# barronalex/Tacotron

Hardware: AMD Instinct MI355X
Metric: mel-frames/sec (train step, batch=32 r=2) (higher is better)
Workload: dtype f32

## Files before the change

### include/taco_hip.h

```cpp
#ifndef TACO_HIP_H
#define TACO_HIP_H

#include <stddef.h>
#include <stdint.h>

#ifdef __cplusplus
extern "C" {
#endif
#pragma GCC visibility push(default)

#define TACO_VERSION 120

#define TACO_OK 0
#define TACO_EINVAL (-1)
#define TACO_ELAUNCH (-2)
#define TACO_ENOTFOUND (-3)

#define TACO_ACT_NONE 0
#define TACO_ACT_RELU 1
#define TACO_ACT_SIGMOID 2
#define TACO_ACT_TANH 3

typedef struct TacoShape {
  int32_t B;
// ... 109 lines not shown
                  float* grads, void* workspace, void* stream);

int taco_infer(const TacoShape* shape, const float* params, const int32_t* text, const int32_t* text_length,
               const int32_t* speaker,
               float* seq2seq_output, float* output, float* alignments, void* workspace, void* stream);

typedef struct TacoStopRule {
  int32_t end_offset;
  int32_t hold;
  int32_t min_steps;
  int32_t reserved;
} TacoStopRule;

int taco_infer_stop(const TacoShape* shape, const float* params, const int32_t* text, const int32_t* text_length,
                    const int32_t* speaker, const TacoStopRule* rule, float* seq2seq_output, float* output, float* alignments,
                    int32_t* lengths, void* workspace, void* stream);

#define TACO_ALIGNMENT_MAX_TD 16384
#define TACO_ALIGNMENT_MAX_TT 16384
int taco_alignment_scores(const float* alignments, const int32_t* text_length, const int32_t* steps, int max_jump,
                          int32_t* counts, float* means, int B, int Td, int Tt, void* stream);

#define TACO_ALIGN_PATH_MAX_TD   16384
#define TACO_ALIGN_PATH_MAX_TT   4096
#define TACO_ALIGN_PATH_MAX_JUMP 15
int64_t taco_alignment_path_workspace_bytes(int B, int Td, int Tt);
int taco_alignment_path(const float* alignments, const int32_t* text_length, const int32_t* steps, int max_jump,
                        int32_t* path, int32_t* dur, int32_t* counts, float* mass, void* workspace,
                        int B, int Td, int Tt, void* stream);

int taco_frames_active(const float* x, float floor, int32_t* n, int B, int F, int C, void* stream);

#define TACO_DTW_MAX_FRAMES 1024
#define TACO_DTW_MAX_K 32
#define TACO_DTW_MAX_C 128
int64_t taco_frame_dtw_workspace_bytes(int B, int Fa, int Fb, int K);
int taco_frame_dtw(const float* a, const int32_t* na, const float* b, const int32_t* nb, const float* basis, float* cost,
                   int32_t* steps, void* workspace, int B, int Fa, int Fb, int C, int K, void* stream);

int64_t taco_frame_dtw_path_workspace_bytes(int B, int Fa, int Fb, int K);
int taco_frame_dtw_path(const float* a, const int32_t* na, const float* b, const int32_t* nb, const float* basis, float* cost,
                        int32_t* steps, int32_t* path_a, int32_t* path_b, void* workspace, int B, int Fa, int Fb, int C, int K,
                        void* stream);

int taco_clip_adam_step(float* params, const float* grads, float* m, float* v, int64_t n, float lr, float cap,
                        int64_t step, float* scratch, float* gnorm_out, void* stream);

int taco_clip_adam_step_guarded(float* params, const float* grads, float* m, float* v, int64_t n, float lr, float cap,
                                int64_t step, float* scratch, float* gnorm_out, const int32_t* err_words, void* stream);
int taco_clear_error(const TacoShape* shape, int train, void* workspace, void* stream);

int taco_decoder_mode(int mode);

int taco_grad_segments(const TacoShape* shape, int64_t* bounds);
int taco_wait_grad_segment(int seg, void* stream);
int taco_debug_spin(int blocks, int threads, int lds_bytes, int usec, void* stream);

int taco_debug_clock_probe(long long* out3, int iters, void* stream);

int taco_debug_fabric_probe(long long* out32, void* gran4k, const void* scratch, long long scratch_bytes, int iters, void* stream);

int taco_denorm_unframe(const float* output, const float* stft_mean, const float* stft_std, float* spec, float* mag_t,
                        int B, int Td, int r, int C, void* stream);

#define TACO_STRETCH_ONE        65536
#define TACO_STRETCH_MIN_STEP   16384
#define TACO_STRETCH_MAX_STEP   262144
#define TACO_STRETCH_MAX_FRAMES 8192
int taco_frames_stretch(const float* mag_t, const int32_t* frames, int frames_per_unit, const int32_t* step_q,
                        float* out, int32_t* frames_out, int B, int C, int F, int Fo, void* stream);

#define TACO_PITCH_ONE        65536
#define TACO_PITCH_MIN_STEP   32768
#define TACO_PITCH_MAX_STEP   131072
#define TACO_PITCH_MAX_LIFTER 64
#define TACO_PITCH_FLOOR      1e-8f
int taco_frames_pitch(const float* mag_t, const int32_t* frames, int frames_per_unit, const int32_t* step_q, int lifter,
                      float* out, int B, int C, int F, void* stream);

int taco_path_curve(const int32_t* path, const int32_t* values, int frames_per_step, int32_t fill, int32_t* curve, int B, int Td,
                    int Tt, void* stream);
int taco_frames_stretch_curve(const float* mag_t, const int32_t* frames, int frames_per_unit, const int32_t* dur_q, float* out,
                              int32_t* frames_out, int32_t* src, int B, int C, int F, int Fo, void* stream);
int taco_frames_pitch_curve(const float* mag_t, const int32_t* frames, int frames_per_unit, const int32_t* step_q, int lifter,
                            float* out, int B, int C, int F, void* stream);

#define TACO_SHARPEN_FIRST    2
#define TACO_SHARPEN_MIN_BETA -1.0f
#define TACO_SHARPEN_MAX_BETA 1.0f
int taco_frames_sharpen(const float* mag_t, const int32_t* frames, int frames_per_unit, float beta, int lifter, float* out, int B,
                        int C, int F, void* stream);
int64_t taco_frames_cepstats_workspace_bytes(int B, int C, int F, int lifter);
int taco_frames_cepstats(const float* mag_t, const int32_t* frames, int frames_per_unit, int lifter, double* sums, int32_t* count,
                         void* workspace, int B, int C, int F, void* stream);

#define TACO_F0_MAX_LAGS 512
int taco_frames_f0(const float* mag_t, const int32_t* frames, int frames_per_unit, const float* weight, const float* gain,
                   int lag_min, int lag_max, float ratio, float threshold, float* period, float* strength, float* acf,
                   int B, int C, int F, void* stream);

int taco_f0_stats(const float* period, const float* other, const int32_t* frames, int frames_per_unit, float* stats, int B, int F,
                  void* stream);

#define TACO_F0_MAX_CAND 15
int64_t taco_f0_viterbi_workspace_bytes(int B, int L, int F, int K);
int taco_f0_viterbi(const float* acf, const int32_t* frames, int frames_per_unit, const float* bias, const float* lg, int lag_min,
// ... 76 lines not shown
```

### tacotron_amd/csrc/gemm.hip

```cpp
#include <algorithm>

#include "bf16x3.h"
#include "common.h"
#include "kernels.h"

namespace {

constexpr int BK = 16;

__device__ __forceinline__ float4 sel4(bool ok, const float4 t) {
  return make_float4(ok ? t.x : 0.f, ok ? t.y : 0.f, ok ? t.z : 0.f, ok ? t.w : 0.f);
}

struct RowInfo {
  int m;
  int t;
  bool ok;
};

template <int WM, int WN, bool VA, bool VB>
__global__ __launch_bounds__(256) void conv_gemm_kernel(ConvGemmBatch batch) {
  constexpr int BM = 64 * WM, BN = 64 * WN;
  constexpr int LDS_A = BM + 4, LDS_B = BN + 4;
  constexpr int A_PER = BM / 64;
  constexpr int B_PER = BN / 64;
  const ConvGemmProblem& P = batch.p[blockIdx.z];
  const int m0 = blockIdx.x * BM, n0 = blockIdx.y * BN;
  if (m0 >= P.M || n0 >= P.N) return;

  __shared__ __attribute__((aligned(16))) float As[2][BK][LDS_A];
  __shared__ __attribute__((aligned(16))) float Bs[2][BK][LDS_B];

  const int tid = threadIdx.x, lane = tid & 63, wave = tid >> 6;
  const int wm = wave >> 1, wn = wave & 1;

  const int a_kq = tid & 3;
  const int a_row = tid >> 2;
  RowInfo ar[A_PER];
#pragma unroll
  for (int i = 0; i < A_PER; ++i) {
    int m = m0 + a_row + 64 * i;
    ar[i].m = m;
    ar[i].ok = m < P.M;
    ar[i].t = ar[i].ok ? (m % P.T) : 0;
  }
  constexpr int B_COLS4 = BN / 4;
  const int b_c4 = tid % B_COLS4;
  const int b_k = tid / B_COLS4;
  constexpr int B_KSTEP = 256 / B_COLS4;

  const int ktiles = (P.K + BK - 1) / BK;
  const int nit = P.taps * ktiles;

// ... 381 lines not shown
      if (kk + 2 < BK) {
#pragma unroll
        for (int i = 0; i < WM; ++i) a[nxt][i] = As[buf][kk + 2 + lk][wm * (32 * WM) + i * 32 + li];
#pragma unroll
        for (int j = 0; j < WN; ++j) b[nxt][j] = Bs[buf][kk + 2 + lk][wn * (32 * WN) + j * 32 + li];
      }
#pragma unroll
      for (int i = 0; i < WM; ++i)
#pragma unroll
        for (int j = 0; j < WN; ++j)
          acc[i][j] = __builtin_amdgcn_mfma_f32_32x32x2f32(a[cur][i], b[cur][j], acc[i][j], 0, 0, 0);
    }
    if (it + 1 < nit) store_tile(buf ^ 1);
    __syncthreads();
  }

  if constexpr (BX) {
#pragma unroll
    for (int i = 0; i < WM; ++i)
#pragma unroll
      for (int j = 0; j < WN; ++j) acc[i][j] += acc_lo[i][j];
  }
#pragma unroll
  for (int i = 0; i < WM; ++i) {
#pragma unroll
    for (int j = 0; j < WN; ++j) {
      const int n = n0 + wn * (32 * WN) + j * 32 + li;
      if (n >= P.N) continue;
#pragma unroll
      for (int e = 0; e < 16; ++e) {
        const int k = k0 + wm * (32 * WM) + i * 32 + (e & 3) + 8 * (e >> 2) + 4 * lk;
        if (k >= P.K) continue;
        atomicAdd(&W[(int64_t)k * P.ldw + n], acc[i][j][e]);
      }
    }
  }
  if (do_bias) {
    float* cs = &As[0][0][0];
    float4 t = make_float4(0.f, 0.f, 0.f, 0.f);
#pragma unroll
    for (int i = 0; i < B_PER; ++i) { t.x += bsum[i].x; t.y += bsum[i].y; t.z += bsum[i].z; t.w += bsum[i].w; }
    __syncthreads();
    *reinterpret_cast<float4*>(&cs[b_r * LDS_B + b_c4 * 4]) = t;
    __syncthreads();
    float* db = P.dbias + (int64_t)bz * P.N;
    for (int i = tid; i < BN; i += 256) {
      float c = 0.f;
      for (int r = 0; r < B_RSTEP; ++r) c += cs[r * LDS_B + i];
      if (n0 + i < P.N) atomicAdd(&db[n0 + i], c);
    }
  }
}

__device__ __forceinline__ void tn_xcd_order(int L, int per, int gz, bool on, int& t, int& z) {
  const int zfull = gz & ~7;
  if (on && L < per * zfull) {
    const int x = L & 7, s = L >> 3;
    const int g = s / per;
    z = x + 8 * g;
    t = s - g * per;
  } else {
    z = L / per;
    t = L - z * per;
  }
}

template <int WM, int WN, bool VA, bool VB, bool BX = false>
__global__ __launch_bounds__(256) void gemm_tn_kernel(GemmTnArgs P) {
  const int gx = gridDim.x, per = gx * gridDim.y;
  int t, z;
  tn_xcd_order(blockIdx.x + gx * (blockIdx.y + gridDim.y * blockIdx.z), per, gridDim.z, P.xcd != 0, t, z);
  const int by = t / gx;
  gemm_tn_body<WM, WN, VA, VB, BX>(P, t - by * gx, by, z);
}

template <bool BX>
__global__ __launch_bounds__(256) void gemm_tn_batch_kernel(GemmTnBatch B) {
  int pi = 0;
  for (int i = 1; i < B.n; ++i)
    if ((int)blockIdx.x >= B.first[i]) pi = i;
  const GemmTnArgs& P = B.p[pi];
  const int rel = blockIdx.x - B.first[pi];
  const int gx = B.gx[pi], per = gx * B.gy[pi], gz = P.batch * P.taps * P.splits;
  if (rel >= per * gz) return;
  int t, z;
  tn_xcd_order(rel, per, gz, P.xcd != 0, t, z);
  const int by = t / gx;
  gemm_tn_body<1, 1, true, true, BX>(P, t - by * gx, by, z);
}

__global__ void gemm_naive_kernel(ConvGemmProblem P) {
  const int64_t idx = (int64_t)blockIdx.x * blockDim.x + threadIdx.x;
  if (idx >= (int64_t)P.M * P.N) return;
  const int m = (int)(idx / P.N), n = (int)(idx % P.N);
  const int t = m % P.T;
  float acc = 0.f;
  for (int tap = 0; tap < P.taps; ++tap) {
    const int st = t + tap - P.pad_l;
    if (st < 0 || st >= P.T) continue;
    const float* a = P.A + (int64_t)(m + tap - P.pad_l) * P.lda;
    const float* w = P.W + (int64_t)tap * P.K * P.ldw + n;
    for (int k = 0; k < P.K; ++k) acc = fmaf(a[k], w[(int64_t)k * P.ldw], acc);
  }
  if (P.bias) acc += P.bias[n];
  P.C[(int64_t)m * P.ldc + n] = apply_act(acc, P.act);
}

inline bool aligned16(const void* p) { return (reinterpret_cast<uintptr_t>(p) & 15) == 0; }

}

void conv_gemm_set_flags(ConvGemmProblem& p) {
  p.flags = 0;
  if (p.Nld <= 0) p.Nld = (p.N % 4 == 0) ? p.N : 0;
  if (p.lda % 4 == 0 && aligned16(p.A) && p.K % 4 == 0) p.flags |= 1;
  if (p.ldw % 4 == 0 && aligned16(p.W) && ((int64_t)p.K * p.ldw) % 4 == 0 && p.Nld > 0 && p.Nld % 4 == 0 && p.Nld <= p.ldw)
    p.flags |= 2;
}

template <int WM, int WN>
static void dispatch_nn(int flags, dim3 grid, hipStream_t s, ConvGemmBatch& batch) {
  switch (flags & 3) {
    case 3: TACO_KLAUNCH((conv_gemm_kernel<WM, WN, true, true>), grid, dim3(256), 0, s, batch); break;
    case 1: TACO_KLAUNCH((conv_gemm_kernel<WM, WN, true, false>), grid, dim3(256), 0, s, batch); break;
    case 2: TACO_KLAUNCH((conv_gemm_kernel<WM, WN, false, true>), grid, dim3(256), 0, s, batch); break;
    default: TACO_KLAUNCH((conv_gemm_kernel<WM, WN, false, false>), grid, dim3(256), 0, s, batch); break;
  }
}

int launch_conv_gemm_batch(ConvGemmBatch& batch, hipStream_t stream) {
  TACO_REQUIRE(batch.n >= 1 && batch.n <= kMaxGemmBatch, "conv_gemm: batch size %d out of range", batch.n);
  int maxM = 0, maxN = 0, flags = 3;
  double work = 0;
  for (int i = 0; i < batch.n; ++i) {
    ConvGemmProblem& p = batch.p[i];
    TACO_REQUIRE(p.A && p.W && p.C, "conv_gemm: null operand");
    TACO_REQUIRE(p.M > 0 && p.N > 0 && p.K > 0 && p.taps > 0 && p.T > 0, "conv_gemm: bad dims M=%d N=%d K=%d taps=%d T=%d",
                 p.M, p.N, p.K, p.taps, p.T);
    TACO_REQUIRE(p.M % p.T == 0, "conv_gemm: M (%d) must be a multiple of T (%d)", p.M, p.T);
    conv_gemm_set_flags(p);
    flags &= p.flags;
// ... 75 lines not shown
          ConvGemmProblem& r = b.p[c];
          r = ConvGemmProblem();
          r.A = p.A; r.lda = p.lda; r.W = p.W; r.ldw = p.ldw; r.Nld = p.Nld; r.C = slabs + c * mn; r.ldc = p.N;
          r.M = p.M; r.N = p.N; r.K = p.K; r.taps = p.taps; r.T = p.T; r.pad_l = p.pad_l; r.act = TACO_ACT_NONE;
          r.it0 = c * per;
          r.it1 = std::min(nit, (c + 1) * per);
          conv_gemm_set_flags(r);
        }
        const int pslot = taco_prof_begin(2, stream);
        taco_prof_label(2, pslot, "nn-ksplit S=%d M=%d N=%d K=%d taps=%d", bestS, p.M, p.N, p.K, p.taps);
        const int rc = launch_conv_gemm2(b, stream, true);
        if (rc == TACO_OK) {
          const int64_t total4 = mn / 4;
          const int grid = (int)((total4 + 255) / 256 > 2048 ? 2048 : (total4 + 255) / 256);
          TACO_KLAUNCH(conv_gemm_tapsum_kernel, dim3(grid), dim3(256), 0, stream, p, slabs, bestS);
          taco_prof_end(2, pslot, stream, 2.0 * p.M * p.N * p.K * p.taps);
          TACO_LAUNCH_CHECK("conv_gemm2 k-split");
          return TACO_OK;
        }
        taco_prof_cancel(2, pslot, stream);
        if (rc != TACO_ENOTFOUND) return rc;
      }
    }
  }
  const double tiles64 = (double)cdiv(p.M, 64) * cdiv(p.N, 64);
  if (!slabs || p.taps < 2 || p.taps > kMaxGemmBatch || p.N % 4 != 0 || p.atomic_out || tiles64 > 320 || p.K < 512)
    return launch_conv_gemm(p, stream);
  ConvGemmBatch b;
  b.n = p.taps;
  const int64_t slab = (int64_t)p.M * p.N;
  for (int t = 0; t < p.taps; ++t) {
    ConvGemmProblem q;
    q.A = p.A; q.lda = p.lda; q.W = p.W + (int64_t)t * p.K * p.ldw; q.ldw = p.ldw; q.Nld = p.Nld;
    q.C = slabs + t * slab; q.ldc = p.N;
    q.M = p.M; q.N = p.N; q.K = p.K; q.taps = 1; q.T = p.T; q.pad_l = p.pad_l - t;
    q.act = TACO_ACT_NONE;
    b.p[t] = q;
  }
  TACO_TRY(launch_conv_gemm_batch(b, stream));
  const int64_t total4 = slab / 4;
  const int grid = (int)((total4 + 255) / 256 > 2048 ? 2048 : (total4 + 255) / 256);
  TACO_KLAUNCH(conv_gemm_tapsum_kernel, dim3(grid), dim3(256), 0, stream, p, slabs, p.taps);
  TACO_LAUNCH_CHECK("conv_gemm_tapsum");
  return TACO_OK;
}

int launch_conv_gemm(const ConvGemmProblem& p, hipStream_t stream) {
  ConvGemmBatch b;
  b.n = 1;
  b.p[0] = p;
  return launch_conv_gemm_batch(b, stream);
}

template <int WM, int WN>
static void dispatch_tn(int flags, dim3 grid, hipStream_t s, const GemmTnArgs& a) {
  switch (flags & 3) {
    case 3:
      if (env_bf16x() && a.chunk <= bf16x_max_chain()) TACO_KLAUNCH((gemm_tn_kernel<WM, WN, true, true, true>), grid, dim3(256), 0, s, a);
      else TACO_KLAUNCH((gemm_tn_kernel<WM, WN, true, true>), grid, dim3(256), 0, s, a);
      break;
    case 1: TACO_KLAUNCH((gemm_tn_kernel<WM, WN, true, false>), grid, dim3(256), 0, s, a); break;
    case 2: TACO_KLAUNCH((gemm_tn_kernel<WM, WN, false, true>), grid, dim3(256), 0, s, a); break;
    default: TACO_KLAUNCH((gemm_tn_kernel<WM, WN, false, false>), grid, dim3(256), 0, s, a); break;
  }
}

static int tn_block_target() {
  const int x = sw_int<SW_TN_BLOCKS>();
  return x > 0 ? x : 3072;
}

static int plan_gemm_tn(GemmTnArgs& a, bool force_small, dim3& grid, int64_t group_tiles = 0) {
  a.flags = 0;
  if (a.Nld <= 0) a.Nld = (a.N % 4 == 0) ? a.N : 0;
  const int64_t lim31 = (int64_t)1 << 31;
  if (a.lda % 4 == 0 && aligned16(a.A) && a.strideA % 4 == 0 && a.K % 4 == 0 && ((int64_t)a.M + a.taps + 48) * a.lda * 4 < lim31)
    a.flags |= 1;
  if (a.ldy % 4 == 0 && aligned16(a.Y) && a.strideY % 4 == 0 && a.Nld > 0 && a.Nld % 4 == 0 && a.Nld <= a.ldy &&
      ((int64_t)a.M + 16) * a.ldy * 4 < lim31)
    a.flags |= 2;
  const bool merge_taps = sw_on<SW_TN_MERGE_TAPS>();
  if (merge_taps && a.ktap == 0 && (a.flags & 1) && a.taps > 1 && a.taps <= 17 && a.K % 64 != 0 && a.pad_l <= 16 && a.taps - 1 - a.pad_l <= 16) {
    a.ktap = a.K;
    a.K *= a.taps;
    a.taps = 1;
  }
  const int force_bm = sw_int<SW_TN_BM>(), big_tiles = sw_int<SW_TN_BIG_TILES>();
  bool big = !force_small && (int64_t)cdiv(a.K, 128) * cdiv(a.N, 128) * a.taps * a.batch >= big_tiles && a.K >= 128 && a.N >= 128;
  if (!force_small && force_bm == 128 && a.K >= 128 && a.N >= 128) big = true;
  if (force_bm == 64) big = false;
  const int bm = big ? 128 : 64;
  const int64_t tiles = (int64_t)cdiv(a.K, bm) * cdiv(a.N, bm) * a.taps * a.batch;
  const int64_t fill = group_tiles > tiles ? group_tiles : tiles;
  int splits = taco_deterministic() ? 1 : (int)((tn_block_target() + fill - 1) / fill);
  const int max_splits = a.M >= 1280 ? cdiv(a.M, 320) : cdiv(a.M, 64);
  if (splits > max_splits) splits = max_splits;
  if (splits < 1) splits = 1;
  int chunk = cdiv(a.M, splits);
  chunk = cdiv(chunk, BK) * BK;
  splits = cdiv(a.M, chunk);
  a.splits = splits;
  a.chunk = chunk;
  grid = dim3(cdiv(a.K, bm), cdiv(a.N, bm), a.batch * a.taps * splits);
  a.xcd = sw_int<SW_TN_XCD>();
  return bm;
}

int launch_gemm_tn(GemmTnArgs a, bool zero_first, hipStream_t stream) {
  TACO_REQUIRE(a.A && a.Y && a.W, "gemm_tn: null operand");
  TACO_REQUIRE(a.M > 0 && a.N > 0 && a.K > 0 && a.taps > 0 && a.T > 0 && a.batch > 0, "gemm_tn: bad dims");
  TACO_REQUIRE(a.M % a.T == 0, "gemm_tn: M (%d) must be a multiple of T (%d)", a.M, a.T);
// ... 31 lines not shown
  TACO_REQUIRE(b.n >= 0 && b.n <= kMaxTnBatch, "gemm_tn_batch: %d problems out of range", b.n);
  GemmTnBatch grouped;
  int blocks = 0;
  GemmTnArgs big[kMaxTnBatch];
  int nbig = 0;
  double big_flops = 0;
  int64_t group_tiles = 0;
  for (int i = 0; i < b.n; ++i) {
    dim3 grid;
    GemmTnArgs probe = b.p[i];
    if (probe.A && probe.M > 0 && probe.N > 0 && probe.K > 0 && probe.taps > 0 && probe.batch > 0 && !gemm_tn2_eligible(probe) &&
        plan_gemm_tn(probe, false, grid) == 64 && probe.flags == 3)
      group_tiles += (int64_t)grid.x * grid.y * probe.taps * probe.batch;
  }
  for (int i = 0; i < b.n; ++i) {
    GemmTnArgs a = b.p[i];
    TACO_REQUIRE(a.A && a.Y && a.W, "gemm_tn_batch: null operand");
    TACO_REQUIRE(a.M > 0 && a.N > 0 && a.K > 0 && a.taps > 0 && a.T > 0 && a.batch > 0 && a.M % a.T == 0, "gemm_tn_batch: bad dims");
    if (gemm_tn2_eligible(a)) {
      big[nbig++] = a;
      big_flops += 2.0 * a.M * a.N * a.K * a.taps;
      continue;
    }
    dim3 grid;
    GemmTnArgs probe = a;
    const int bm = plan_gemm_tn(probe, false, grid, group_tiles);
    if (bm == 128 || probe.flags != 3) {
      TACO_TRY(launch_gemm_tn(a, false, stream));
      continue;
    }
    const int j = grouped.n++;
    grouped.p[j] = probe;
    grouped.first[j] = blocks;
    grouped.gx[j] = (int)grid.x;
    grouped.gy[j] = (int)grid.y;
    blocks += (int)(grid.x * grid.y * grid.z);
    blocks = (blocks + 7) & ~7;
  }
  if (nbig > 0) {
    const int pslot = taco_prof_begin(2, stream);
    TACO_TRY(launch_gemm_tn2(big, nbig, stream));
    taco_prof_end(2, pslot, stream, big_flops);
    TACO_LAUNCH_CHECK("gemm_tn2 batch");
  }
  if (grouped.n > 0) {
    double flops = 0;
    for (int i = 0; i < grouped.n; ++i)
      flops += 2.0 * grouped.p[i].M * grouped.p[i].N * grouped.p[i].K * grouped.p[i].taps * grouped.p[i].batch;
    const int pslot = taco_prof_begin(2, stream);
    taco_prof_label(2, pslot, "tn-batch n=%d blocks=%d first: M=%d N=%d K=%d taps=%d", grouped.n, blocks, grouped.p[0].M, grouped.p[0].N, grouped.p[0].K,
                    grouped.p[0].taps);
    int max_chunk = 0;
    for (int i = 0; i < grouped.n; ++i) max_chunk = grouped.p[i].chunk > max_chunk ? grouped.p[i].chunk : max_chunk;
    if (env_bf16x() && max_chunk <= bf16x_max_chain()) TACO_KLAUNCH(gemm_tn_batch_kernel<true>, dim3(blocks), dim3(256), 0, stream, grouped);
    else TACO_KLAUNCH(gemm_tn_batch_kernel<false>, dim3(blocks), dim3(256), 0, stream, grouped);
    taco_prof_end(2, pslot, stream, flops);
    TACO_LAUNCH_CHECK("gemm_tn_batch");
  }
  b.n = 0;
  return TACO_OK;
}

int launch_gemm_naive(const ConvGemmProblem& p, hipStream_t stream) {
  const int64_t n = (int64_t)p.M * p.N;
  TACO_KLAUNCH(gemm_naive_kernel, dim3(cdiv(n, 256)), dim3(256), 0, stream, p);
  TACO_LAUNCH_CHECK("gemm_naive");
  return TACO_OK;
}


extern "C" int taco_debug_conv_gemm_batch_atomic(const float* dbank, int lda, const float* const* WT, const float* residual, int ldr,
                                                 float* dx_out, int ldc, int M, int T, int F, int K, int N, void* stream) {
  const char* who = "taco_debug_conv_gemm_batch_atomic";
  TACO_REQUIRE(M > 0 && M <= kDoorMaxRows, "%s: M must be in [1, 2^22], got %d", who, M);
  TACO_REQUIRE(T > 0 && M % T == 0, "%s: T must be positive and divide M = %d, got %d", who, M, T);
  TACO_REQUIRE(F >= 1 && F <= kMaxGemmBatch, "%s: F must be in [1, %d], got %d", who, kMaxGemmBatch, F);
  TACO_REQUIRE(N > 0 && N <= kDoorMaxCols, "%s: N must be in [1, 2^14], got %d", who, N);
  TACO_REQUIRE(K > 0 && K <= kDoorMaxCols, "%s: K must be in [1, 2^14], got %d", who, K);
  TACO_REQUIRE(lda >= F * K, "%s: lda must be >= F K = %d, got %d", who, F * K, lda);
  TACO_REQUIRE(ldc >= N, "%s: ldc must be >= N = %d, got %d", who, N, ldc);
  TACO_REQUIRE(!residual || ldr >= N, "%s: ldr must be >= N = %d, got %d", who, N, ldr);
  TACO_REQUIRE(WT, "%s: WT is null", who);
  DoorOperands o;
  o.in(dbank, door_span(M, (int64_t)F * K, lda), "dbank");
  for (int f = 1; f <= F; ++f) o.in(WT[f - 1], (size_t)f * K * N * sizeof(float), "WT[%d]", f - 1);
  o.in_opt(residual, door_span(M, N, ldr), "residual");
  o.out(dx_out, door_span(M, N, ldc), "dx_out");
  TACO_TRY(o.check(who));
  ConvGemmBatch batch;
  batch.n = F;
  for (int k = 1; k <= F; ++k) {
    ConvGemmProblem& p = batch.p[F - k];
    p = ConvGemmProblem();
    p.A = dbank + (k - 1) * K; p.lda = lda; p.W = WT[k - 1]; p.ldw = N; p.C = dx_out; p.ldc = ldc; p.M = M; p.N = N;
    p.K = K; p.taps = k; p.T = T; p.pad_l = (k - 1) - (k - 1) / 2; p.act = TACO_ACT_NONE; p.atomic_out = 1;
    if (k == 1) {
      p.residual = residual;
      p.ldr = ldr;
    }
  }
  return launch_conv_gemm_batch(batch, as_stream(stream));
}

extern "C" int taco_debug_conv_gemm_rowbias(const float* A, int lda, const float* W, int ldw, const float* rowb, int bias_stride, float* C,
                                            int ldc, int M, int T, int N, int K, void* stream) {
  const char* who = "taco_debug_conv_gemm_rowbias";
  TACO_REQUIRE(M > 0 && M <= kDoorMaxRows, "%s: M must be in [1, 2^22], got %d", who, M);
// ... 83 lines not shown
```

### tacotron_amd/lib.py

```python
from __future__ import annotations

import collections
import ctypes as C
import math
import os

from . import QUEUES_SET_BY_USER as _QUEUES_SET_BY_USER, TORCH_IMPORTED_FIRST as _TORCH_IMPORTED_FIRST

import numpy as np
import torch

from .argcheck import (float_arg, int_arg, no_overlap, on_gpu, pow2_bins, step_q_arg, tensor_arg,
                       host_int32 as _host_int32, own_or_given as _own_or_given, unit_interval as _unit_interval)

HW_QUEUES_LATE = (not _QUEUES_SET_BY_USER) and (_TORCH_IMPORTED_FIRST or (torch.cuda.is_available() and torch.cuda.is_initialized()))


def effective_hw_queues() -> int:
    if HW_QUEUES_LATE:
        return 4
    try:
        return int(os.environ.get('GPU_MAX_HW_QUEUES', '4'))
    except ValueError:
        return 4
# ... 55 lines not shown
    'taco_debug_conv_gemm_ksplit': (C.c_int, [_P, _I, _P, _I, _P, _P, _I, _I, _I, _I, _I, _I, _I, _I, _P, C.c_int64, _P]),
    'taco_gemm_tn': (C.c_int, [_P, _I, _P, _I, _P, _I, _I, _I, _I, _I, _I, _I, _I, _P]),
    'taco_debug_gemm_naive': (C.c_int, [_P, _I, _P, _I, _P, _P, _I, _I, _I, _I, _I, _I, _I, _I, _P]),
    'taco_bigru_fwd': (C.c_int, [_P] * 12 + [_I, _I, _P]),
    'taco_debug_bigru_rec_fwd': (C.c_int, [_P] * 8 + [_I, _I, _P]),
    'taco_debug_bigru_bwd': (C.c_int, [_P] * 11 + [_I, _I, _P]),
    'taco_debug_highway_stack_fwd': (C.c_int, [_P] * 10 + [_I, _I, _I, _P]),
    'taco_debug_highway_stack_bwd': (C.c_int, [_P] * 8 + [_I, _I, _P]),
    'taco_debug_prenet_fwd': (C.c_int, [_P] * 9 + [_I, _P]),
    'taco_debug_prenet_bwd': (C.c_int, [_P] * 10 + [_I, _P]),
    'taco_debug_conv_bank_pool_fwd': (C.c_int, [_P, _I, _P, _P, _P, _P, C.c_float, _P, _P, _I, _I, _I, _I, _I, _I, _P]),
    'taco_debug_conv_gemm_pool_bwd': (C.c_int, [_P, _I, _P, _I, _P, _P, _P, C.c_float, _P, _I, _P, _P, _I, _I, _I, _I, _I, _I, _P]),
    'taco_debug_bn_maxpool_fwd': (C.c_int, [_P] * 4 + [_I, _I, _I, _P]),
    'taco_debug_bn_maxpool_bwd': (C.c_int, [_P] * 7 + [_I, _I, _I, _P]),
    'taco_debug_bank_gather': (C.c_int, [_P, _I, _P, _P, _I, _P, _I, _P, C.c_int64, _I, _I, _I, _I, _I, _I, _I, _P]),
    'taco_debug_conv_gemm_batch_atomic': (C.c_int, [_P, _I, _P, _P, _I, _P, _I, _I, _I, _I, _I, _I, _P]),
    'taco_debug_conv_gemm_rowbias': (C.c_int, [_P, _I, _P, _I, _P, _I, _P, _I, _I, _I, _I, _I, _P]),
    'taco_debug_gemm_tn_group': (C.c_int, [_I] + [_P] * 13 + [_P]),
    'taco_debug_gemm_tn_strided': (C.c_int, [_P, _I, C.c_int64, _P, _I, C.c_int64, _P, _I, C.c_int64, _I, _I, _I, _I, _I, _I, _P]),
    'taco_debug_embedding': (C.c_int, [_P, _P, _P, _I, _I, _I, _P]),
    'taco_debug_embedding_bwd': (C.c_int, [_P, _P, _P, _I, _I, _I, _P]),
    'taco_debug_highway_combine': (C.c_int, [_P, _P, _P, _I, _P]),
    'taco_debug_highway_combine_bwd': (C.c_int, [_P] * 5 + [_I, _P]),
    'taco_debug_act_bwd': (C.c_int, [_P, _P, _P, _P, C.c_int64, _I, _P]),
    'taco_debug_affine_act_bwd': (C.c_int, [_P] * 6 + [_I, _I, _I, _P]),
    'taco_debug_colsum_batched': (C.c_int, [_P, _I, _P, _I, _I, _I, _P]),
    'taco_debug_mask_rows': (C.c_int, [_P, _P, _P, _I, _I, _I, _P]),
    'taco_debug_center_rows': (C.c_int, [_P, _P, _P, _I, _I, _I, _P]),
    'taco_debug_mask_pos': (C.c_int, [_P, _I, _P, _I, _I, _I, C.c_float, _P]),
    'taco_debug_zero_tail_rows': (C.c_int, [_P, _I, _P, _I, _P, _I, _I, _P]),
    'taco_debug_add': (C.c_int, [_P, _P, _P, C.c_int64, _P]),
    'taco_debug_l1_loss': (C.c_int, [_P, _P, _P, _I, _I, _I, _P, _P, _P, _I, _I, _I, _P, _P, _P, _P]),
    'taco_debug_transpose_batch': (C.c_int, [_I] + [_P] * 7 + [_P]),
    'taco_debug_sumsq': (C.c_int, [_P, C.c_int64, _P, _P]),
    'taco_forward': (C.c_int, [_SH] + [_P] * 17),
    'taco_backward': (C.c_int, [_SH] + [_P] * 14),
    'taco_infer': (C.c_int, [_SH] + [_P] * 9),
    'taco_infer_stop': (C.c_int, [_SH, _P, _P, _P, _P, C.POINTER(TacoStopRule), _P, _P, _P, _P, _P, _P]),
    'taco_alignment_scores': (C.c_int, [_P, _P, _P, _I, _P, _P, _I, _I, _I, _P]),
    'taco_alignment_path_workspace_bytes': (C.c_int64, [_I, _I, _I]),
    'taco_alignment_path': (C.c_int, [_P, _P, _P, _I, _P, _P, _P, _P, _P, _I, _I, _I, _P]),
    'taco_frames_active': (C.c_int, [_P, C.c_float, _P, _I, _I, _I, _P]),
    'taco_frame_dtw_workspace_bytes': (C.c_int64, [_I, _I, _I, _I]),
    'taco_frame_dtw': (C.c_int, [_P, _P, _P, _P, _P, _P, _P, _P, _I, _I, _I, _I, _I, _P]),
    'taco_frame_dtw_path_workspace_bytes': (C.c_int64, [_I, _I, _I, _I]),
    'taco_frame_dtw_path': (C.c_int, [_P, _P, _P, _P, _P, _P, _P, _P, _P, _P, _I, _I, _I, _I, _I, _P]),
    'taco_path_f0_scores': (C.c_int, [_P, _P, _P, _P, _P, C.c_float, _P, _P, _I, _I, _I, _P]),
    'taco_clip_adam_step': (C.c_int, [_P, _P, _P, _P, C.c_int64, C.c_float, C.c_float, C.c_int64, _P, _P, _P]),
    'taco_clip_adam_step_guarded': (C.c_int, [_P, _P, _P, _P, C.c_int64, C.c_float, C.c_float, C.c_int64, _P, _P, _P, _P]),
    'taco_clear_error': (C.c_int, [_SH, _I, _P, _P]),
    'taco_grad_segments': (C.c_int, [_SH, C.POINTER(C.c_int64)]),
    'taco_wait_grad_segment': (C.c_int, [_I, _P]),
    'taco_decoder_mode': (C.c_int, [_I]),
    'taco_debug_spin': (C.c_int, [_I, _I, _I, _I, _P]),
    'taco_debug_clock_probe': (C.c_int, [_P, _I, _P]),
    'taco_debug_fabric_probe': (C.c_int, [_P, _P, _P, C.c_int64, _I, _P]),
    'taco_denorm_unframe': (C.c_int, [_P, _P, _P, _P, _P, _I, _I, _I, _I, _P]),
    'taco_frames_stretch': (C.c_int, [_P, _P, _I, _P, _P, _P, _I, _I, _I, _I, _P]),
    'taco_frames_pitch': (C.c_int, [_P, _P, _I, _P, _I, _P, _I, _I, _I, _P]),
    'taco_path_curve': (C.c_int, [_P, _P, _I, C.c_int32, _P, _I, _I, _I, _P]),
    'taco_frames_stretch_curve': (C.c_int, [_P, _P, _I, _P, _P, _P, _P, _I, _I, _I, _I, _P]),
    'taco_frames_pitch_curve': (C.c_int, [_P, _P, _I, _P, _I, _P, _I, _I, _I, _P]),
    'taco_frames_sharpen': (C.c_int, [_P, _P, _I, C.c_float, _I, _P, _I, _I, _I, _P]),
    'taco_frames_cepstats_workspace_bytes': (C.c_int64, [_I, _I, _I, _I]),
    'taco_frames_cepstats': (C.c_int, [_P, _P, _I, _I, _P, _P, _P, _I, _I, _I, _P]),
    'taco_frames_f0': (C.c_int, [_P, _P, _I, _P, _P, _I, _I, C.c_float, C.c_float, _P, _P, _P, _I, _I, _I, _P]),
    'taco_f0_stats': (C.c_int, [_P, _P, _P, _I, _P, _I, _I, _P]),
    'taco_f0_viterbi_workspace_bytes': (C.c_int64, [_I, _I, _I, _I]),
    'taco_f0_viterbi': (C.c_int, [_P, _P, _I, _P, _P, _I, _I, _I, C.c_float, C.c_float, C.c_float, _P, _P, _P, _P, _P, _I, _I, _P]),
    'taco_corpus_batch': (C.c_int, [_P, _I, _P, _P, _P, _P, _P, C.c_int64, _I, C.c_int64, _I, _P]),
    'taco_griffinlim_workspace_bytes': (C.c_int64, [_I, _I]),
    'taco_griffinlim': (C.c_int, [_P, _P, _P, _P, _I, _I, _I, _P]),
    'taco_griffinlim_rows_workspace_bytes': (C.c_int64, [_I, _I]),
    'taco_griffinlim_rows': (C.c_int, [_P, _P, C.c_uint64, _P, _I, _P, _P, _I, _I, _I, _P]),
    'taco_griffinlim_fast_workspace_bytes': (C.c_int64, [_I, _I]),
    'taco_griffinlim_fast': (C.c_int, [_P, _P, C.c_uint64, _P, _I, C.c_float, _P, _P, _P, _I, _I, _I, _P]),
    'taco_phase_estimate_workspace_bytes': (C.c_int64, [_I, _I]),
    'taco_phase_estimate': (C.c_int, [_P, _P, _I, _P, _P, _I, _I, _P]),
    'taco_wave_finish_workspace_bytes': (C.c_int64, [_I, _I]),
    'taco_wave_finish': (C.c_int, [_P, _P, C.c_float, C.c_float, _P, _P, _P, _P, _P, _I, _I, _P]),
    'taco_wave_join_workspace_bytes': (C.c_int64, [_I, _I, _I]),
    'taco_wave_join': (C.c_int, [_P, C.c_int64, _P, C.POINTER(C.c_int32), C.POINTER(C.c_int32), _I, _P, _P, _P, _P, _P, _P, _I, _I, _I, _I,
                                 _P]),
    'taco_k_weighting': (C.c_int, [_I, C.POINTER(C.c_double)]),
    'taco_wave_loudness_workspace_bytes': (C.c_int64, [_I, _I, _I]),
    'taco_wave_loudness': (C.c_int, [_P, _P, _I, C.c_float, C.c_float, _P, _P, _P, _P, _P, _I, _I, _P]),
    'taco_wave_limit_workspace_bytes': (C.c_int64, [_I, _I, _I]),
    'taco_wave_limit': (C.c_int, [_P, _P, _P, C.c_float, _P, _I, _I, _P, _I, _P, _P, _P, _P, _P, _I, _I, _P]),
    'taco_audio_features_workspace_bytes': (C.c_int64, [_I, _I]),
    'taco_audio_features': (C.c_int, [_P, C.POINTER(C.c_int32), _P, _P, _P, _P, _P, _P, _I, _I, _I, _I, _I, _P]),
    'taco_wave_resample': (C.c_int, [_P, C.c_int64, _I, _I, _P, _P, _I, _I, _I, _I, _P, _I, _I, _P]),
    'taco_fill_bernoulli': (C.c_int, [_P, C.c_int64, C.c_float, C.c_uint64, _P]),
    'taco_tensor_stats_plan_bytes': (C.c_int64, [C.POINTER(C.c_int64), _I]),
    'taco_tensor_stats_plan': (C.c_int, [C.POINTER(C.c_int64), _I, C.c_int64, _P, C.c_int64, C.POINTER(C.c_int32)]),
    'taco_tensor_stats_workspace_bytes': (C.c_int64, [_I, _I, _I]),
    'taco_tensor_stats': (C.c_int, [_P, _P, _P, _I, _I, _I, _I, _I, _P, _P, _P, _P, _P]),
    'taco_profile_enable': (C.c_int, [_I]),
    'taco_debug_last_cluster': (C.c_int, [_I]),
    'taco_profile_read': (C.c_int, [_I, C.POINTER(C.c_float), _I]),
    'taco_debug_profile_labels': (C.c_int, [_I, C.c_char_p, _I]),
    'taco_profile_read2': (C.c_int, [_I, C.POINTER(C.c_float), C.POINTER(C.c_double), _I]),
}
for _name, (_res, _args) in EXPORTS.items():
    _fn = getattr(_lib, _name)
    _fn.restype = _res
    _fn.argtypes = _args
# ... 729 lines not shown
    return int_arg(who, 'B', B, 1, _INT_MAX), int_arg(who, 'Td', Td, 1), int_arg(who, 'Tt', Tt, 1)


def alignment_path_workspace_bytes(B, Td, Tt) -> int:
    return _size('taco_alignment_path_workspace_bytes', *_path_shape('alignment_path_workspace_bytes', B, Td, Tt))


def alignment_path(alignments, text_length, steps=None, max_jump=PATH_JUMP, path=None, dur=None, counts=None, mass=None, workspace=None):
    who = 'alignment_path'
    B, Td, Tt = tensor_arg(who, 'alignments', alignments, torch.float32, ('B', 'Td', 'Tt'))
    dev = alignments.device
    _path_shape(who, B, Td, Tt)
    tensor_arg(who, 'text_length', text_length, torch.int32, (B,), dev)
    tensor_arg(who, 'steps', steps, torch.int32, (B,), dev, optional=True)
    max_jump = int_arg(who, 'max_jump', max_jump, 1, PATH_MAX_JUMP)
    path = _own_or_given(path, (B, Td), torch.int32, dev, who + ': path')
    dur = _own_or_given(dur, (B, Tt), torch.int32, dev, who + ': dur')
    counts = _own_or_given(counts, (B, len(PATH_COUNTS)), torch.int32, dev, who + ': counts')
    mass = _own_or_given(mass, (B,), torch.float32, dev, who + ': mass')
    if workspace is not None:
        tensor_arg(who, 'workspace', workspace, torch.uint8, ('bytes',), dev, empty_ok=True)
    on_gpu(who, 'alignments', dev)
    workspace = _own_or_given(workspace, (alignment_path_workspace_bytes(B, Td, Tt),), torch.uint8, dev, who + ': workspace')
    _check(_lib.taco_alignment_path(ptr(alignments), ptr(text_length), ptr(steps), max_jump, ptr(path), ptr(dur), ptr(counts), ptr(mass),
                                    ptr(workspace) if workspace.numel() else None, B, Td, Tt, stream_ptr()), 'taco_alignment_path')
    return path, dur, counts, mass


def clip_adam_step(params, grads, m, v, lr, cap, step, scratch, gnorm_out, err_words=None):
    assert scratch.numel() >= 256, 'taco: clip_adam scratch must hold 256 floats'
    _check(_lib.taco_clip_adam_step_guarded(ptr(params), ptr(grads), ptr(m), ptr(v), params.numel(), float(lr), float(cap),
                                            int(step), ptr(scratch), ptr(gnorm_out), ptr(err_words), stream_ptr()),
           'taco_clip_adam_step_guarded')


def clear_error(shape, train, workspace):
    _check(_lib.taco_clear_error(C.byref(shape), int(train), ptr(workspace), stream_ptr()), 'taco_clear_error')


def grad_segments(shape):
    b = (C.c_int64 * 8)()
    n = _lib.taco_grad_segments(C.byref(shape), b)
    if n < 1 or n > 7:
        raise TacoError('taco_grad_segments: ' + last_error())
    return [int(x) for x in b[:n + 1]]


def wait_grad_segment(seg, stream):
    _check(_lib.taco_wait_grad_segment(int(seg), C.c_void_p(stream.cuda_stream)), 'taco_wait_grad_segment')


def decoder_mode(mode=-1) -> int:
    return _lib.taco_decoder_mode(int(mode))


def clock_probe(iters=1 << 20):
    out = torch.zeros(3, dtype=torch.int64, device='cuda')
    for _ in range(2):
        _check(_lib.taco_debug_clock_probe(ptr(out), int(iters), stream_ptr()), 'taco_debug_clock_probe')
    torch.cuda.synchronize()
    cyc, ticks = out[0].item(), out[1].item()
    return cyc / (ticks * 10.0) if ticks > 0 else 0.0


def fabric_probe(iters=2000, scratch_mb=768):
    out = torch.zeros(32, dtype=torch.int64, device='cuda')
    gran = torch.zeros(512, dtype=torch.int64, device='cuda')
    scratch = torch.zeros(scratch_mb << 18, dtype=torch.int32, device='cuda')
    res = None
    for _ in range(2):
        out.zero_(); gran.zero_()
        _check(_lib.taco_debug_fabric_probe(ptr(out), ptr(gran), ptr(scratch), int(scratch.numel() * 4), int(iters), stream_ptr()),
               'taco_debug_fabric_probe')
        torch.cuda.synchronize()
        res = out.tolist()
    n = max(1, res[6])
    ok = res[7]
    xcc = res[8:32]
    hop = lambda t: t * 10.0 / n / 2.0
    return {'hop_ns_same_xcd_l2_local': hop(res[0]) if ok & 1 else None,
            'hop_ns_same_xcd_agent_scope': hop(res[1]) if ok & 2 else None,
            'hop_ns_cross_xcd': hop(res[2]) if ok & 4 else None,
            'load_ns_l2_hit': res[3] * 10.0 / n, 'load_ns_agent_scope_cold': res[4] * 10.0 / n,
            'one_cu_stream_gb_s': (8 << 20) / (res[5] * 10e-9) / 1e9 if res[5] > 0 else None,
            'xcc_of_pairs': {'l2_local': [xcc[0], xcc[8]], 'agent': [xcc[1], xcc[9]], 'cross': [xcc[2], xcc[3]]},
            'scratch_mb': scratch_mb}


def debug_spin(blocks, threads, lds_bytes, usec, stream=None):
    sp = stream_ptr() if stream is None else C.c_void_p(stream.cuda_stream)
    _check(_lib.taco_debug_spin(int(blocks), int(threads), int(lds_bytes), int(usec), sp), 'taco_debug_spin')


def denorm_unframe(output, stft_mean, stft_std, r, want_spec=True, want_mag_t=False, spec=None, mag_t=None):
    B, Td, RC = output.shape
    Cw = RC // r
    F = (Td // 4) * 4 * r
    spec = _own_or_given(spec, (B, F, Cw), torch.float32, output.device, 'denorm_unframe: spec') if want_spec else None
    mag_t = _own_or_given(mag_t, (B, Cw, F), torch.float32, output.device, 'denorm_unframe: mag_t') if want_mag_t else None
    _check(_lib.taco_denorm_unframe(ptr(output), ptr(stft_mean), ptr(stft_std), ptr(spec), ptr(mag_t), B, Td, r, Cw,
                                    stream_ptr()), 'taco_denorm_unframe')
    if want_spec and want_mag_t:
        return spec, mag_t
    return spec if want_spec else mag_t


# ... 1040 lines not shown
```

Baseline: 1.593 million.

## Add stage-split bf16x3 TN gemm body with per-wave load/split roles

```diff
diff --git a/include/taco_hip.h b/include/taco_hip.h
--- a/include/taco_hip.h
+++ b/include/taco_hip.h
@@ -185,6 +185,8 @@
 
 int taco_decoder_mode(int mode);
 
+int taco_tn_stage_split(int on);
+
 int taco_grad_segments(const TacoShape* shape, int64_t* bounds);
 int taco_wait_grad_segment(int seg, void* stream);
 int taco_debug_spin(int blocks, int threads, int lds_bytes, int usec, void* stream);
diff --git a/tacotron_amd/csrc/gemm.hip b/tacotron_amd/csrc/gemm.hip
--- a/tacotron_amd/csrc/gemm.hip
+++ b/tacotron_amd/csrc/gemm.hip
@@ -1,4 +1,5 @@
 #include <algorithm>
+#include <type_traits>
 
 #include "bf16x3.h"
 #include "common.h"
@@ -486,6 +487,157 @@
   }
 }
 
+__device__ __forceinline__ void gemm_tn_body_ss(const GemmTnArgs& P, const int bx, const int by, const int bz_) {
+  static_assert(BK == 16, "one v_mfma_f32_32x32x16_bf16 group per 16-row tile");
+  const int k0 = bx * 64, n0 = by * 64;
+  int z = bz_;
+  const int split = z % P.splits;
+  z /= P.splits;
+  const int tap = z % P.taps;
+  const int bz = z / P.taps;
+  const float* A = P.A + (int64_t)bz * P.strideA;
+  const float* Y = P.Y + (int64_t)bz * P.strideY;
+  float* W = P.W + (int64_t)bz * P.strideW + (int64_t)tap * P.K * P.ldw;
+
+  __shared__ __attribute__((aligned(16))) u32x4 Ps[2][2][3][2][64];
+
+  const int tid = threadIdx.x, lane = tid & 63;
+  const int wave = __builtin_amdgcn_readfirstlane(tid >> 6);
+  const int wm = wave >> 1, wn = wave & 1;
+  const int s_op = wave >> 1, s_lk = wave & 1;
+
+  const int m_begin = split * P.chunk;
+  const int m_end = min(P.M, m_begin + P.chunk);
+  const int nit = (m_end - m_begin + BK - 1) / BK;
+  if (nit <= 0) return;
+  const bool do_bias = P.dbias != nullptr && bx == 0 && tap == 0;
+  float bsum = 0.f;
+
+  constexpr int kOOB = (int)0x80000000;
+  const int sh_u = s_op == 0 ? tap - P.pad_l : 0;
+  int sh_t = sh_u;
+  int vo;
+  if (s_op == 0) {
+    const int k = k0 + lane;
+    int kcol = k;
+    if (P.ktap > 0) {
+      const int tc = k / P.ktap;
+      kcol -= tc * P.ktap;
+      sh_t = tc - P.pad_l;
+    }
+    vo = k < P.K ? ((m_begin + s_lk + sh_t + 16) * P.lda + kcol) * 4 : kOOB;
+  } else {
+    const int n = n0 + lane;
+    vo = n < P.Nld ? ((m_begin + s_lk) * P.ldy + n) * 4 : kOOB;
+  }
+  const __amdgpu_buffer_rsrc_t rs = __builtin_amdgcn_make_buffer_rsrc(
+      const_cast<float*>(s_op == 0 ? A - (int64_t)16 * P.lda : Y), 0, 0x7fffffff, 0x00020000);
+  const __amdgpu_buffer_rsrc_t rs0 = __builtin_amdgcn_make_buffer_rsrc(
+      const_cast<float*>(s_op == 0 ? A - (int64_t)16 * P.lda : Y), 0, 0, 0x00020000);
+  const int ld4 = (s_op == 0 ? P.lda : P.ldy) * 4;
+  int t0 = m_begin % P.T;
+  const int t_step = BK % P.T;
+  const int sh_lo = s_op == 0 && P.ktap > 0 ? -P.pad_l : sh_u;
+  const int sh_hi = s_op == 0 && P.ktap > 0 ? P.K / P.ktap - 1 - P.pad_l : sh_u;
+  const bool sum_cols = do_bias && s_op == 1;
+
+  auto load_frag = [&](int it, float (&r)[8]) {
+    const int row0 = it * BK;
+    const int t = t0;
+    t0 += t_step;
+    t0 = t0 >= P.T ? t0 - P.T : t0;
+    if (m_begin + row0 + BK <= m_end && t + BK <= P.T && t + sh_lo >= 0 && t + BK - 1 + sh_hi < P.T) {
+#pragma unroll
+      for (int q = 0; q < 8; ++q) r[q] = __builtin_bit_cast(float, __builtin_amdgcn_raw_buffer_load_b32(rs, vo, (row0 + 2 * q) * ld4, 0));
+    } else if (P.ktap > 0) {
+#pragma unroll
+      for (int q = 0; q < 8; ++q) {
+        const int m = m_begin + row0 + 2 * q + s_lk;
+        const bool ok = m < m_end && (unsigned)(m % P.T + sh_t) < (unsigned)P.T;
+        r[q] = __builtin_bit_cast(float, __builtin_amdgcn_raw_buffer_load_b32(rs, ok ? vo : kOOB, (row0 + 2 * q) * ld4, 0));
+      }
+    } else {
+#pragma unroll
+      for (int q = 0; q < 8; ++q) {
+        const int m = m_begin + row0 + 2 * q + s_lk;
+        const bool ok = m < m_end && (unsigned)(m % P.T + sh_u) < (unsigned)P.T;
+        r[q] = __builtin_bit_cast(float, __builtin_amdgcn_raw_buffer_load_b32(ok ? rs : rs0, vo, (row0 + 2 * q) * ld4, 0));
+      }
+    }
+  };
+  auto split_frag = [&](const float (&r)[8]) {
+    const float s = ((((((r[0] + r[1]) + r[2]) + r[3]) + r[4]) + r[5]) + r[6]) + r[7];
+    bsum += sum_cols ? s : 0.f;
+    return split8(r[0], r[1], r[2], r[3], r[4], r[5], r[6], r[7]);
+  };
+  auto store_frag = [&](int buf, const Pl3& p) {
+    Ps[buf][s_op][0][s_lk][lane] = p.h;
+    Ps[buf][s_op][1][s_lk][lane] = p.m;
+    Ps[buf][s_op][2][s_lk][lane] = p.l;
+  };
+
+  f32x16 acc, acc_lo;
+#pragma unroll
+  for (int e = 0; e < 16; ++e) acc[e] = acc_lo[e] = 0.f;
+
+  float f[8], g[8];
+  load_frag(0, f);
+  load_frag(1, g);
+  store_frag(0, split_frag(f));
+  load_frag(2, f);
+  __syncthreads();
+  const int lk = lane >> 5, li = lane & 31;
+  auto tile = [&](int it, float (&r)[8], auto more_c) __attribute__((always_inline)) {
+    constexpr bool more = decltype(more_c)::value;
+    const int buf = it & 1;
+    Pl3 pa, pb;
+    pa.l = Ps[buf][0][2][lk][wm * 32 + li];
+    pb.h = Ps[buf][1][0][lk][wn * 32 + li];
+    pa.h = Ps[buf][0][0][lk][wm * 32 + li];
+    pb.l = Ps[buf][1][2][lk][wn * 32 + li];
+    pa.m = Ps[buf][0][1][lk][wm * 32 + li];
+    pb.m = Ps[buf][1][1][lk][wn * 32 + li];
+    mfma6_2(acc, acc_lo, pa, pb);
+    if constexpr (more) {
+      Pl3 pn = split_frag(r);
+#pragma unroll
+      for (int i = 0; i < 6; ++i) {
+        __builtin_amdgcn_sched_group_barrier(0x8, 1, 0);
+        __builtin_amdgcn_sched_group_barrier(0x2, 9, 0);
+      }
+      asm volatile("" : "+v"(pn.h), "+v"(pn.m), "+v"(pn.l), "+v"(bsum));
+      __builtin_amdgcn_sched_barrier(0);
+      load_frag(it + 3, r);
+      store_frag(buf ^ 1, pn);
+    }
+    __syncthreads();
+  };
+  int it = 0;
+  for (; it + 2 < nit; it += 2) {
+    tile(it, g, std::true_type{});
+    tile(it + 1, f, std::true_type{});
+  }
+  if (it + 1 < nit) tile(it++, g, std::true_type{});
+  tile(it, f, std::false_type{});
+
+  acc += acc_lo;
+  const int n = n0 + wn * 32 + li;
+  if (n < P.N) {
+#pragma unroll
+    for (int e = 0; e < 16; ++e) {
+      const int k = k0 + wm * 32 + (e & 3) + 8 * (e >> 2) + 4 * lk;
+      if (k >= P.K) continue;
+      atomicAdd(&W[(int64_t)k * P.ldw + n], acc[e]);
+    }
+  }
+  if (do_bias) {
+    float* cs = reinterpret_cast<float*>(&Ps[0][0][0][0][0]);
+    if (s_op == 1) cs[s_lk * 64 + lane] = bsum;
+    __syncthreads();
+    if (tid < 64 && n0 + tid < P.N) atomicAdd(&P.dbias[(int64_t)bz * P.N + n0 + tid], cs[tid] + cs[64 + tid]);
+  }
+}
+
 __device__ __forceinline__ void tn_xcd_order(int L, int per, int gz, bool on, int& t, int& z) {
   const int zfull = gz & ~7;
   if (on && L < per * zfull) {
@@ -499,16 +651,18 @@
   }
 }
 
-template <int WM, int WN, bool VA, bool VB, bool BX = false>
+template <int WM, int WN, bool VA, bool VB, bool BX = false, bool SS = false>
 __global__ __launch_bounds__(256) void gemm_tn_kernel(GemmTnArgs P) {
+  static_assert(!SS || (WM == 1 && WN == 1 && VA && VB && BX), "the stage-split form is the 64 x 64 bf16x3 vector kernel");
   const int gx = gridDim.x, per = gx * gridDim.y;
   int t, z;
   tn_xcd_order(blockIdx.x + gx * (blockIdx.y + gridDim.y * blockIdx.z), per, gridDim.z, P.xcd != 0, t, z);
   const int by = t / gx;
-  gemm_tn_body<WM, WN, VA, VB, BX>(P, t - by * gx, by, z);
-}
-
-template <bool BX>
+  if constexpr (SS) gemm_tn_body_ss(P, t - by * gx, by, z);
+  else gemm_tn_body<WM, WN, VA, VB, BX>(P, t - by * gx, by, z);
+}
+
+template <bool BX, bool SS = false>
 __global__ __launch_bounds__(256) void gemm_tn_batch_kernel(GemmTnBatch B) {
   int pi = 0;
   for (int i = 1; i < B.n; ++i)
@@ -520,7 +674,8 @@
   int t, z;
   tn_xcd_order(rel, per, gz, P.xcd != 0, t, z);
   const int by = t / gx;
-  gemm_tn_body<1, 1, true, true, BX>(P, t - by * gx, by, z);
+  if constexpr (SS) gemm_tn_body_ss(P, t - by * gx, by, z);
+  else gemm_tn_body<1, 1, true, true, BX>(P, t - by * gx, by, z);
 }
 
 __global__ void gemm_naive_kernel(ConvGemmProblem P) {
@@ -702,11 +857,26 @@
   return launch_conv_gemm_batch(b, stream);
 }
 
+static int g_tn_stage_split = 1;
+extern "C" int taco_tn_stage_split(int on) {
+  const int prev = g_tn_stage_split;
+  if (on >= 0) g_tn_stage_split = on != 0;
+  return prev;
+}
+
 template <int WM, int WN>
 static void dispatch_tn(int flags, dim3 grid, hipStream_t s, const GemmTnArgs& a) {
   switch (flags & 3) {
     case 3:
-      if (env_bf16x() && a.chunk <= bf16x_max_chain()) TACO_KLAUNCH((gemm_tn_kernel<WM, WN, true, true, true>), grid, dim3(256), 0, s, a);
+      if (env_bf16x() && a.chunk <= bf16x_max_chain()) {
+        if constexpr (WM == 1 && WN == 1) {
+          if (g_tn_stage_split) {
+            TACO_KLAUNCH((gemm_tn_kernel<1, 1, true, true, true, true>), grid, dim3(256), 0, s, a);
+            break;
+          }
+        }
+        TACO_KLAUNCH((gemm_tn_kernel<WM, WN, true, true, true>), grid, dim3(256), 0, s, a);
+      }
       else TACO_KLAUNCH((gemm_tn_kernel<WM, WN, true, true>), grid, dim3(256), 0, s, a);
       break;
     case 1: TACO_KLAUNCH((gemm_tn_kernel<WM, WN, true, false>), grid, dim3(256), 0, s, a); break;
@@ -844,7 +1014,9 @@
                     grouped.p[0].taps);
     int max_chunk = 0;
     for (int i = 0; i < grouped.n; ++i) max_chunk = grouped.p[i].chunk > max_chunk ? grouped.p[i].chunk : max_chunk;
-    if (env_bf16x() && max_chunk <= bf16x_max_chain()) TACO_KLAUNCH(gemm_tn_batch_kernel<true>, dim3(blocks), dim3(256), 0, stream, grouped);
+    const bool bx = env_bf16x() && max_chunk <= bf16x_max_chain();
+    if (bx && g_tn_stage_split) TACO_KLAUNCH((gemm_tn_batch_kernel<true, true>), dim3(blocks), dim3(256), 0, stream, grouped);
+    else if (bx) TACO_KLAUNCH(gemm_tn_batch_kernel<true>, dim3(blocks), dim3(256), 0, stream, grouped);
     else TACO_KLAUNCH(gemm_tn_batch_kernel<false>, dim3(blocks), dim3(256), 0, stream, grouped);
     taco_prof_end(2, pslot, stream, flops);
     TACO_LAUNCH_CHECK("gemm_tn_batch");
diff --git a/tacotron_amd/lib.py b/tacotron_amd/lib.py
--- a/tacotron_amd/lib.py
+++ b/tacotron_amd/lib.py
@@ -131,6 +131,7 @@
     'taco_grad_segments': (C.c_int, [_SH, C.POINTER(C.c_int64)]),
     'taco_wait_grad_segment': (C.c_int, [_I, _P]),
     'taco_decoder_mode': (C.c_int, [_I]),
+    'taco_tn_stage_split': (C.c_int, [_I]),
     'taco_debug_spin': (C.c_int, [_I, _I, _I, _I, _P]),
     'taco_debug_clock_probe': (C.c_int, [_P, _I, _P]),
     'taco_debug_fabric_probe': (C.c_int, [_P, _P, _P, C.c_int64, _I, _P]),
@@ -966,6 +967,10 @@
 
 def decoder_mode(mode=-1) -> int:
     return _lib.taco_decoder_mode(int(mode))
+
+
+def tn_stage_split(on=-1) -> int:
+    return _lib.taco_tn_stage_split(int(on))
 
 
 def clock_probe(iters=1 << 20):
```

Measured after the change: 1.606 million (median of 6 runs). No clear change (+0.8%).
